# NickQrumpton/lattice-gaussian-mcmc

Hardware: AMD Instinct MI355X
Metric: Klein samples/sec at n=512 NTRU (IMHK proposals, d=1024) (higher is better)
Workload: dtype f64

## Files before the change

include/lgs.h:

```cpp
#ifndef LGS_H
#define LGS_H

#include <stdint.h>

#ifdef __cplusplus
extern "C" {
#endif

#define LGS_OK 0
#define LGS_ERR_INVALID (-1)
#define LGS_ERR_HIP (-2)
#define LGS_ERR_NOMEM (-3)
#define LGS_ERR_OVERFLOW (-4)
#define LGS_ERR_NONFINITE (-5)
#define LGS_ERR_STATE (-6)

#define LGS_BASIS_LINEAR_PROBS 0x1u

#define LGS_DEVICE_PTRS 0x1u
#define LGS_EXACT_ORDER 0x2u
#define LGS_WANG_LING 0x4u
#define LGS_Z64 0x8u
#define LGS_COORD_MAJOR 0x10u
#define LGS_SAMPLEZ_TABLE 0x20u
// ... 118 lines not shown
int lgs_timing_get(lgs_ctx *ctx, int kernel, double *ms_total, int64_t *launches);

#define LGS_COUNTER_RESOLVED 0
#define LGS_COUNTER_FALLBACK 1
#define LGS_COUNTER_ACCEPT_RESOLVED 2
#define LGS_COUNTER_WL_MISMATCH 3
#define LGS_COUNTER_QSKIP 4
#define LGS_COUNTER_KLEIN_CUS 5
#define LGS_COUNTER_DECODE_RESOLVED 6
#define LGS_COUNTER_LAUNCH_EXACT 7
#define LGS_COUNTER_LAUNCH_VALU 8
#define LGS_COUNTER_LAUNCH_MFMA_FP64 9
#define LGS_COUNTER_LAUNCH_MFMA_I8 10
int lgs_counter(lgs_ctx *ctx, int which, int reset, uint64_t *value);

int lgs_device_info(lgs_ctx *ctx, char *name, int name_len, int *n_cu, int64_t *hbm_bytes);

#ifdef __cplusplus
}
#endif
#endif
```

lattice-gaussian-mcmc_amd/csrc/lgs_capi.hip:

```cpp
#include <hip/hip_runtime.h>

#include <algorithm>
#include <cmath>
#include <cstdarg>
#include <cstdio>
#include <cstdlib>
#include <climits>
#include <cstring>
#include <string>
#include <vector>

#include "../../include/lgs.h"
#include "lgs_kernels.h"
#include "lgs_szc_host.h"

namespace {

thread_local std::string g_err;

int fail(int code, const char* fmt, ...) {
    char buf[512];
    va_list ap;
    va_start(ap, fmt);
    vsnprintf(buf, sizeof(buf), fmt, ap);
    va_end(ap);
    g_err = buf;
    return code;
}
// ... 14 lines not shown
static bool hook_is(const char* name, int v) {
    const char* e = hook(name);
    return e && atoi(e) == v;
}

#ifdef LGS_TEST_HOOKS
static size_t test_nomem_above() {
    const char* e = hook("LGS_TEST_NOMEM_ABOVE");
    return e ? (size_t)atoll(e) : 0;
}
#endif

struct DevBuf {
    void* p = nullptr;
    size_t bytes = 0;
    ~DevBuf() {
        if (p) (void)hipFree(p);
    }
    int reserve(size_t need) {
        if (need <= bytes) return LGS_OK;
        if (p) {
            (void)hipFree(p);
            p = nullptr;
            bytes = 0;
        }
        if (need == 0) return LGS_OK;
#ifdef LGS_TEST_HOOKS
        if (test_nomem_above() && need > test_nomem_above())
            return fail(LGS_ERR_NOMEM, "hipMalloc(%zu) refused (LGS_TEST_NOMEM_ABOVE)", need);
#endif
        hipError_t e = hipMalloc(&p, need);
        if (e != hipSuccess) {
            p = nullptr;
            return fail(LGS_ERR_NOMEM, "hipMalloc(%zu) failed: %s", need, hipGetErrorString(e));
        }
        bytes = need;
        return LGS_OK;
    }
    void release() {
        if (p) (void)hipFree(p);
        p = nullptr;
        bytes = 0;
    }
    template <typename T>
    T* as() const {
        return (T*)p;
    }
};

struct Timer {
    int kernel;
// ... 21 lines not shown
    int64_t d = 0;
    double sigma = 0;
    int precision = 10;
    uint32_t basis_flags = 0;
    int panel = 32;
    bool has_B = false;
    DevBuf R, RP, RC, BT, coord;
    DevBuf CREC, RX;
    DevBuf CERT;
    uint64_t n_resolved = 0;
    DevBuf RT, LWE, EMAX;
    DevBuf QZ2;
    bool has_qz2 = false;
    uint64_t n_accept_resolved = 0, n_wl_mismatch = 0;
    uint64_t n_qskip = 0;
    uint64_t n_decode_resolved = 0;
    uint64_t n_fallback = 0;
    uint64_t n_launch[4] = {};
    double z1cap = 0.0, z1seen = 0.0;
    unsigned int resolved_seen = 0;
    DevBuf RD, RDOFF;
    bool has_rd = false, oz_off = false;
    DevBuf H16, F0;
    DevBuf ZNZ;
    DevBuf CLIVE;
    DevBuf VNP;
    DevBuf LAGP;
    struct {
        const void* Z = nullptr;
        int64_t lanes = 0, cols = 0;
// ... 20 lines not shown
    int zint = 2;
    bool timing = false;
    double t_ms[9] = {0, 0, 0, 0, 0, 0, 0, 0, 0};
    int64_t t_n[9] = {0, 0, 0, 0, 0, 0, 0, 0, 0};
    DevBuf dg_x, dg_y, dg_out, dg_a, dg_b, dg_c, dg_t;
    DevBuf DQ, DBIT;
    DevBuf CPT;
    DevBuf DEC_D, DEC_E, DEC_WIN, DEC_BEST, DEC_D2, DEC_Z;
    bool has_q = false, has_binv = false;
    std::vector<Timer> pending;
    std::vector<hipEvent_t> pool;
    unsigned int* fw_host = nullptr;
    hipEvent_t fw_ev = nullptr;
    struct BlockSet {
        DevBuf Z, LW, H16, ZNZ, CLIVE, flags;
        hipEvent_t ev_free = nullptr;
        bool free_recorded = false;
    } bset[3];
    int bset_next = 0;
    int nsets = 2;
    bool kstream_sets_fixed = false;
    hipStream_t kstream = nullptr;
    hipStream_t kstream_full = nullptr, kstream_split = nullptr;
    int cu_split = 0;
    int kstream_cus = 0;
    int split_cus = 0;
    hipEvent_t kt0 = nullptr, kt1 = nullptr;
    bool kt_pending = false;
    double kt_bz_ms = 0.0;
    hipEvent_t ev_klein = nullptr;
// ... 5 lines not shown
        bool wl = false, exact = false, oz = false;
        decltype(hist) h;
        hipEvent_t ev = nullptr;
    } spec;
};

namespace {

int check_ctx(lgs_ctx* c, bool need_basis = true) {
    if (!c) return fail(LGS_ERR_INVALID, "null context");
    if (need_basis && c->d <= 0) return fail(LGS_ERR_STATE, "no basis loaded (lgs_set_basis)");
    HIP_TRY(hipSetDevice(c->device));
    return LGS_OK;
}

hipEvent_t get_event(lgs_ctx* c) {
    if (!c->pool.empty()) {
        hipEvent_t e = c->pool.back();
        c->pool.pop_back();
        return e;
    }
    hipEvent_t e = nullptr;
    (void)hipEventCreateWithFlags(&e, hipEventDisableSystemFence);
    return e;
}

struct Scope {
    lgs_ctx* c;
    int k;
    hipEvent_t a = nullptr;
// ... 5 lines not shown
    }
    ~Scope() {
        if (c->timing && a) {
            hipEvent_t b = get_event(c);
            (void)hipEventRecord(b, c->stream);
            c->pending.push_back({k, a, b});
        }
    }
};

int run_bz_fp64(lgs_ctx* c, const BzCall& b);

void swap_buf(DevBuf& a, DevBuf& b) {
    std::swap(a.p, b.p);
    std::swap(a.bytes, b.bytes);
}

struct SetSwap {
    lgs_ctx* c = nullptr;
    int j = -1;
    bool flags_in = false, store_in = false;
    void swap_flags() {
        swap_buf(c->flags, c->bset[j].flags);
        flags_in = !flags_in;
    }
    void swap_store() {
        auto& s = c->bset[j];
        swap_buf(c->Z, s.Z);
        swap_buf(c->LW, s.LW);
        swap_buf(c->H16, s.H16);
        swap_buf(c->ZNZ, s.ZNZ);
        swap_buf(c->CLIVE, s.CLIVE);
        store_in = !store_in;
    }
    void restore() {
        if (j < 0) return;
        if (store_in) swap_store();
        if (flags_in) swap_flags();
    }
    bool record = true;
    void release() {
        if (j < 0) return;
        restore();
        if (record) {
            (void)hipEventRecord(c->bset[j].ev_free, c->stream);
            c->bset[j].free_recorded = true;
        }
// ... 12 lines not shown
    const double cost = (double)ms * (double)(ncu - c->split_cus) / (double)c->split_cus;
    if (c->kt_bz_ms > cost) {
        HIP_TRY(hipStreamSynchronize(c->kstream_full));
        c->kstream = c->kstream_split;
        c->kstream_cus = c->split_cus;
        c->cu_split = 1;
    } else {
        c->cu_split = 2;
    }
    return LGS_OK;
}

int spec_discard(lgs_ctx* c) {
    if (!c->spec.valid) return LGS_OK;
    c->spec.valid = false;
    HIP_TRY(hipStreamSynchronize(c->kstream));
    HIP_TRY(hipMemset(c->bset[c->spec.j].flags.p, 0, 4 * lgs::kFlagWords));
    size_t keep = 0;
    for (auto& t : c->pending) {
        if (t.spec) {
            c->pool.push_back(t.a);
            c->pool.push_back(t.b);
        } else {
            c->pending[keep++] = t;
        }
    }
    c->pending.resize(keep);
    return LGS_OK;
}

// ... 51 lines not shown
    }
    c->pending.resize(keep);
}

int finish(lgs_ctx* c, const unsigned int* fw_known = nullptr, bool clear_all = false) {
    int rc0 = settle_bz(c, fw_known);
    if (rc0) return rc0;
    fold_timers(c);
    unsigned int fw[lgs::kFlagWords] = {};
    if (fw_known)
        memcpy(fw, fw_known, sizeof(fw));
    else
        HIP_TRY(hipMemcpy(fw, c->flags.p, sizeof(fw), hipMemcpyDeviceToHost));
    const unsigned int f = fw[0];
    c->resolved_seen = 0;
    if (fw[1] || fw[2] || fw[3])
        fold_counters(c, fw);
    c->n_accept_resolved += fw[lgs::kFlagWordAcceptResolved];
    c->n_wl_mismatch += fw[lgs::kFlagWordWLMismatch];
    c->n_qskip += fw[lgs::kFlagWordQSkip];
    c->n_decode_resolved += fw[lgs::kFlagWordDecodeResolved];
    bool any = false;
    for (int k = 1; k < lgs::kFlagWords; ++k) any |= fw[k] != 0;
    if (clear_all)
        HIP_TRY(hipMemsetAsync(c->flags.p, 0, lgs::kFlagWords * sizeof(unsigned int), c->stream));
    else if (any)
        HIP_TRY(hipMemsetAsync((unsigned int*)c->flags.p + 1, 0, (lgs::kFlagWords - 1) * sizeof(unsigned int),
                               c->stream));
    if (f & lgs::kFlagNonFinite)
        return fail(LGS_ERR_NONFINITE, "non-finite conditional mean (reference raises ValueError)");
    if (f & lgs::kFlagOverflow)
        return fail(LGS_ERR_OVERFLOW, "coefficient |z| >= 2^31: rerun with LGS_Z64");
    return LGS_OK;
}

int finish_or_redo(lgs_ctx* c, bool oz_used, int& zb, bool& redo, bool early = false) {
    redo = false;
    unsigned int fw[lgs::kFlagWords];
    if (early) {
        HIP_TRY(hipEventSynchronize(c->fw_ev));
        memcpy(fw, c->fw_host, sizeof(fw));
    } else {
        HIP_TRY(hipStreamSynchronize(c->stream));
        HIP_TRY(hipMemcpy(fw, c->flags.p, sizeof(fw), hipMemcpyDeviceToHost));
    }
    if (!(fw[0] & lgs::kAbortMask)) return finish(c, fw, early);
    c->pending_i8.clear();
    c->i8_dev_replay = false;
    for (auto& t : c->pending) {
        c->pool.push_back(t.a);
        c->pool.push_back(t.b);
    }
    c->pending.clear();
    c->n_fallback += 1;
    c->n_resolved += fw[kFlagWordCheckpoint];
    if (fw[0] & lgs::kFlagOverflow16) {
        if (zb == 2) c->zint = 4;
        if (oz_used) c->oz_off = true;
    }
    if (fw[0] & lgs::kFlagCarry16) c->zint = 4;
    if (zb == 2) zb = c->zint;
    HIP_TRY(hipMemsetAsync(c->flags.p, 0, 4 * lgs::kFlagWords, c->stream));
    redo = true;
    return LGS_OK;
}

int reset_flags(lgs_ctx* c) {
    int rc = c->flags.reserve(4 * lgs::kFlagWords);
    if (rc) return rc;
    c->resolved_seen = 0;
    HIP_TRY(hipMemsetAsync(c->flags.p, 0, 4 * lgs::kFlagWords, c->stream));
    return LGS_OK;
}

lgs::KleinArgs base_args(lgs_ctx* c, uint64_t seed) {
    lgs::KleinArgs a{};
    const double* co = c->coord.as<double>();
    const int64_t d = c->d;
    a.d = (int)d;
    a.precision = c->precision;
    a.linear_probs = (c->basis_flags & LGS_BASIS_LINEAR_PROBS) ? 1 : 0;
    a.cp = co;
    a.rii = co + d;
    a.sig = co + 2 * d;
// ... 53 lines not shown
        if ((rc = c->ZNZ.reserve((size_t)blocks * lanes))) return rc;
        a.znz = c->ZNZ.as<uint8_t>();
        if (c->d % 16 == 0) {
            const int64_t words = (c->d + 2047) / 2048 * (lanes / 64);
            if ((rc = c->CLIVE.reserve((size_t)words * 4))) return rc;
            HIP_TRY(hipMemsetAsync(c->CLIVE.p, 0, (size_t)words * 4, c->stream));
            a.clive = c->CLIVE.as<unsigned int>();
            a.clive_ld = lanes / 64;
        }
        a.rd = c->RD.as<int8_t>();
        a.rd_off = c->RDOFF.as<int64_t>();
        a.h16 = c->H16.as<int16_t>();
        a.h16_shift = shift;
        a.h16_lanes = lanes;
        used_oz = true;
    }
    const int launched = kernel == lgs::kKernelExact  ? LGS_COUNTER_LAUNCH_EXACT
                         : kernel == lgs::kKernelValu ? LGS_COUNTER_LAUNCH_VALU
                         : used_oz                    ? LGS_COUNTER_LAUNCH_MFMA_I8
                                                      : LGS_COUNTER_LAUNCH_MFMA_FP64;
    c->n_launch[launched - LGS_COUNTER_LAUNCH_EXACT] += 1;
    HIP_TRY(lgs::launch::klein(a, c->R.as<double>(), c->RP.as<double>(), c->RC.as<double>(),
                               c->panel, kernel, wl, zb, Z, c->stream));
    return LGS_OK;
}

int run_klein_store(lgs_ctx* c, lgs::KleinArgs& a, bool exact, bool wl, int& zb, void* Z, bool deferred,
                    bool* oz_out = nullptr) {
    bool oz = false;
    int rc = run_klein(c, a, exact, wl, zb, Z, oz);
// ... 285 lines not shown
    return LGS_OK;
}


int lgs_set_basis(lgs_ctx* c, int64_t d, const double* R, const double* cprime, const double* B,
                  double sigma, int32_t precision, uint32_t flags) {
    int rc = check_ctx(c, false);
    if (rc) return rc;
    if (d <= 0 || d > (1 << 20)) return fail(LGS_ERR_INVALID, "dimension %lld out of range", (long long)d);
    if (!R || !cprime) return fail(LGS_ERR_INVALID, "R and cprime are required");
    if (!(sigma > 0) || !std::isfinite(sigma))
        return fail(LGS_ERR_INVALID, "Standard deviation must be positive, got %g", sigma);
    if (precision <= 0) return fail(LGS_ERR_INVALID, "precision must be positive");
    HIP_TRY(hipStreamSynchronize(c->stream));
    if ((rc = spec_discard(c))) return rc;
    if (c->kstream_split && c->cu_split != 0 && !hook("LGS_PIPE_CU_RESERVE")) {
        HIP_TRY(hipStreamSynchronize(c->kstream));
        c->kstream = c->kstream_full;
        c->kstream_cus = 0;
        c->cu_split = 0;
    }
    c->kt_pending = false;
    const int PB = c->panel;
    const size_t dd = (size_t)d;
    std::vector<double> co(8 * dd);
    for (size_t i = 0; i < dd; ++i) {
        const double rii = R[i * dd + i];
        if (rii == 0.0 || !std::isfinite(rii))
            return fail(LGS_ERR_INVALID, "R[%zu,%zu] must be finite and non-zero", i, i);
        const double sref = sigma / std::fabs(rii);
// ... 366 lines not shown
    const int64_t d = c->d;
    const int zb = z64 ? 8 : 4;
    if ((rc = reset_flags(c))) return rc;
    const void* Zc = z;
    if (!dev || !cm) {
        if ((rc = c->Z.reserve((size_t)n * d * zb)) || (rc = c->stage_a.reserve((size_t)n * d * zb)))
            return rc;
        const void* src = z;
        if (!dev) {
            HIP_TRY(hipMemcpyAsync(c->stage_a.p, z, (size_t)n * d * zb, hipMemcpyHostToDevice, c->stream));
            src = c->stage_a.p;
        }
        if (cm) {
            Zc = src;
        } else {
            HIP_TRY(lgs::launch::to_coord_major(src, zb, n, (int)d, c->Z.p, zb, n, c->stream));
            Zc = c->Z.p;
        }
    }
    double* V = v_out;
    if (!dev) {
        if ((rc = c->V.reserve((size_t)n * d * 8))) return rc;
        V = c->V.as<double>();
    }
    if ((rc = run_bz(c, Zc, zb, n, n, V))) return rc;
    if ((rc = settle_bz(c))) return rc;
    if (!dev) HIP_TRY(hipMemcpyAsync(v_out, V, (size_t)n * d * 8, hipMemcpyDeviceToHost, c->stream));
    return finish(c);
}

// ... 6 lines not shown
    const int64_t d = c->d;
    const int zb = z64 ? 8 : 4;
    if ((rc = reset_flags(c))) return rc;
    const void* Zc = z;
    if (!dev || !cm) {
        if ((rc = c->Z.reserve((size_t)n * d * zb)) || (rc = c->stage_a.reserve((size_t)n * d * zb)))
            return rc;
        const void* src = z;
        if (!dev) {
            HIP_TRY(hipMemcpyAsync(c->stage_a.p, z, (size_t)n * d * zb, hipMemcpyHostToDevice, c->stream));
            src = c->stage_a.p;
        }
        if (cm) {
            Zc = src;
        } else {
            HIP_TRY(lgs::launch::to_coord_major(src, zb, n, (int)d, c->Z.p, zb, n, c->stream));
            Zc = c->Z.p;
        }
    }
    double* o = out;
    if (!dev) {
        if ((rc = c->LW.reserve((size_t)n * 8))) return rc;
        o = c->LW.as<double>();
    }
    lgs::KleinArgs a = base_args(c, 0);
    a.n = n;
    a.ldz = n;
    HIP_TRY(lgs::launch::log_density(a, c->R.as<double>(), Zc, zb, o, c->stream));
    if (!dev) HIP_TRY(hipMemcpyAsync(out, o, (size_t)n * 8, hipMemcpyDeviceToHost, c->stream));
    return finish(c);
// ... 545 lines not shown
        if (value) *value = (uint64_t)c->kstream_cus;
        return LGS_OK;
    }
    uint64_t& v = which >= LGS_COUNTER_LAUNCH_EXACT  ? c->n_launch[which - LGS_COUNTER_LAUNCH_EXACT]
                  : which == LGS_COUNTER_RESOLVED    ? c->n_resolved
                  : which == LGS_COUNTER_FALLBACK    ? c->n_fallback
                  : which == LGS_COUNTER_ACCEPT_RESOLVED ? c->n_accept_resolved
                  : which == LGS_COUNTER_WL_MISMATCH ? c->n_wl_mismatch
                  : which == LGS_COUNTER_DECODE_RESOLVED ? c->n_decode_resolved
                                                     : c->n_qskip;
    if (value) *value = v;
    if (reset) v = 0;
    return LGS_OK;
}

int lgs_device_info(lgs_ctx* c, char* name, int name_len, int* n_cu, int64_t* hbm) {
    int rc = check_ctx(c, false);
    if (rc) return rc;
    hipDeviceProp_t p;
    HIP_TRY(hipGetDeviceProperties(&p, c->device));
    if (name && name_len > 0) {
        snprintf(name, (size_t)name_len, "%s (%s)", p.name, p.gcnArchName);
    }
    if (n_cu) *n_cu = p.multiProcessorCount;
    if (hbm) *hbm = (int64_t)p.totalGlobalMem;
    return LGS_OK;
}

}

// ... 355 lines not shown
            for (int64_t i = 0; i < d; ++i)
                HIP_TRY(hipMemcpyAsync(X + (size_t)i * m, targets + (size_t)i * n + off, (size_t)m * 8,
                                       kind_of(true, dev), c->stream));
        } else {
            const double* src = targets + (size_t)off * d;
            if (!dev) {
                HIP_TRY(hipMemcpyAsync(c->stage_a.p, src, (size_t)m * d * 8, hipMemcpyHostToDevice, c->stream));
                src = c->stage_a.as<double>();
            }
            HIP_TRY(lgs::launch::to_coord_major(src, 8, m, (int)d, X, 8, m, c->stream));
        }
        HIP_TRY(lgs::launch::gemm_f64(X, m, plane ? c->DQ.as<double>() : c->DBIT.as<double>(), (int)d, m, Y,
                                      c->stream));
        HIP_TRY(lgs::launch::to_coord_major(Y, 8, m, (int)d, X, 8, m, c->stream));
        void* Zp = c->Z.p;
        if (plane) {
            const double* co = c->coord.as<double>();
            HIP_TRY(lgs::launch::nearest_plane((int)d, m, c->panel, c->RP.as<double>(), c->RC.as<double>(),
                                               co + d, X, m, ob, Zp, m, c->flags.as<unsigned int>(),
                                               c->stream));
        } else {
            HIP_TRY(lgs::launch::round_coeffs(X, m, (int)d, m, ob, Zp, m, c->flags.as<unsigned int>(),
                                              c->stream));
        }
        if (z_out) {
            if (cm) {
                for (int64_t i = 0; i < d; ++i)
                    HIP_TRY(hipMemcpyAsync((char*)z_out + ((size_t)i * n + off) * ob, (char*)Zp + (size_t)i * m * ob,
                                           (size_t)m * ob, kind_of(dev, true), c->stream));
            } else {
// ... 112 lines not shown
                }
                if (!qframe) {
                    HIP_TRY(lgs::launch::gemm_f64(c->dg_x.as<double>(), m, c->DQ.as<double>(), (int)d, m,
                                                  c->dg_y.as<double>(), c->stream));
                    src = c->dg_y.as<double>();
                }
                HIP_TRY(lgs::launch::to_coord_major(src, 8, m, (int)d, X, 8, mp, c->stream));
            }
        }
        lgs::KleinArgs a = base_args(c, seed);
        a.counter_mode = 0;
        a.base = first + (uint64_t)off;
        a.n = mp;
        a.ldz = mp;
        void* Zp = c->Z.p;
        {
            Scope s(c, 0);
            c->hist.Z = nullptr;
            HIP_TRY(lgs::launch::klein_targets(a, c->R.as<double>(), c->RP.as<double>(), c->RC.as<double>(), c->panel,
                                               exact, X, mp, dmu_scale, ob, Zp, c->stream));
        }
        if (z_out) {
            if (cm) {
                HIP_TRY(hipMemcpy2DAsync((char*)z_out + (size_t)off * ob, (size_t)n * ob, Zp, (size_t)mp * ob,
                                         (size_t)m * ob, (size_t)d, kind_of(dev, true), c->stream));
            } else {
                void* dst = dev ? (char*)z_out + (size_t)off * d * ob : c->stage_a.p;
                HIP_TRY(lgs::launch::transpose_out(Zp, ob, mp, m, (int)d, dst, ob, c->stream));
                if (!dev)
                    HIP_TRY(hipMemcpyAsync((char*)z_out + (size_t)off * d * ob, dst, (size_t)m * d * ob,
// ... 90 lines not shown
                }
                if (!qframe) {
                    HIP_TRY(lgs::launch::gemm_f64(c->dg_x.as<double>(), m, c->DQ.as<double>(), (int)d, m,
                                                  c->dg_y.as<double>(), c->stream));
                    src = c->dg_y.as<double>();
                }
                HIP_TRY(lgs::launch::to_coord_major(src, 8, m, (int)d, X, 8, ldc, c->stream));
            }
        }
        lgs::KleinArgs a = base_args(c, seed);
        a.counter_mode = 0;
        a.base = first + (uint64_t)off * (uint64_t)K;
        a.n = mp;
        a.ldz = mp;
        void* Zp = c->Z.p;
        const lgs::DecodeLanes dl{K, c->DEC_D.as<double>(), c->DEC_E.as<double>()};
        {
            Scope s(c, 0);
            c->hist.Z = nullptr;
            HIP_TRY(lgs::launch::klein_decode(a, c->R.as<double>(), c->RP.as<double>(), c->RC.as<double>(), c->panel,
                                              exact, X, ldc, dmu_scale, ob, Zp, dl, c->stream));
        }
        int64_t* best = dev && o.best_draw ? o.best_draw + off : c->DEC_BEST.as<int64_t>();
        double* dist2 = dev && o.dist2 ? o.dist2 + off : c->DEC_D2.as<double>();
        void* Wp = c->DEC_Z.p;
        {
            Scope s(c, 8);
            HIP_TRY(lgs::launch::decode_select((int)d, m, K, dl.D, dl.E, c->RT.as<double>(), X, ldc, Zp, ob, mp,
                                               c->DEC_WIN.as<int64_t>(), best, dist2, c->flags.as<unsigned int>(),
                                               c->stream, stage_ok));
// ... 44 lines not shown
```

lattice-gaussian-mcmc_amd/csrc/lgs_kernels.h:

```cpp
#pragma once
#include <hip/hip_runtime.h>
#include <stdint.h>


namespace lgs {

constexpr unsigned int kFlagNonFinite = 1u;
constexpr unsigned int kFlagOverflow = 2u;
constexpr unsigned int kFlagI8Range = 4u;
constexpr unsigned int kFlagOverflow16 = 8u;
constexpr unsigned int kFlagCarry16 = 16u;
constexpr unsigned int kAbortMask = kFlagOverflow16 | kFlagCarry16;
constexpr int kFlagWordResolved = 1;
constexpr int kFlagWordUninit = 4;
constexpr int kFlagWordCheckpoint = 5;

constexpr int kErfTabLast = 512;
constexpr int kCoefStride = 18;

constexpr int kSzDeg = 5;
constexpr int kSzS = 9;
constexpr int kSzB = kSzS + kSzDeg + 1;
constexpr int kSzCa = kSzB + kSzDeg + 1;
constexpr int kSzCb = kSzCa + 1;
// ... 54 lines not shown
    const double* cert;
    const double* crec;
    const int8_t* rd;
    const int64_t* rd_off;
    int16_t* h16;
    int h16_shift;
    int64_t h16_lanes;
    uint8_t* znz;
    const double* rx;
    const unsigned int* gate;
    double* LWE;
    unsigned long long* emax;
    const double* qz2;
    unsigned int* clive;
    int64_t clive_ld;
};

constexpr int kFlagWordAcceptResolved = 6;
constexpr int kFlagWordWLMismatch = 7;
constexpr int kFlagWordQSkip = 8;
constexpr int kFlagWordDecodeResolved = 9;
constexpr int kFlagWords = 16;

struct DecodeLanes {
    int64_t K;
    double* D;
    double* E;
};

struct AcceptArgs {
    int64_t nc;
    int64_t T;
    int64_t thin;
    int64_t n_keep;
    uint64_t seed;
    uint32_t chain0;
// ... 150 lines not shown
```

lattice-gaussian-mcmc_amd/csrc/lgs_kernels.hip:

```cpp
#include <hip/hip_runtime.h>

#include <type_traits>
#include <stdint.h>

#include "lgs_device.h"
#include "lgs_kernels.h"

namespace lgs {

typedef unsigned int v4u_t __attribute__((ext_vector_type(4)));

__device__ __forceinline__ void lane_counter(const KleinArgs& a, int64_t p, uint32_t& chain,
                                             uint32_t& step) {
    if (a.counter_mode == 0) {
        const uint64_t s = a.base + (uint64_t)p;
        chain = (uint32_t)s;
        step = (uint32_t)(s >> 32);
    } else {
        chain = a.chain0 + (uint32_t)(p / a.nt);
        step = a.step0 + (uint32_t)(p % a.nt);
    }
}

__device__ __forceinline__ double ref_weight(double zi, double mu, double ros, double isr, double lterm) {
// ... 803 lines not shown
#pragma unroll
    for (int g = 0; g < 4; ++g)
#pragma unroll
        for (int reg = 0; reg < 4; ++reg) F[(4 * h + reg) * LDF + 16 * g + n] = t0v[g][reg];
#ifdef LGS_DIAG_FAR
    {
        LGS_DF_T(tf_end);
        df[7] += 1;
        df[5] += (tf_end - tf_begin) - df[0] - df[1] - df[2] - df[3] - df[4];
        if ((threadIdx.x & 63) == 0)
            for (int k = 0; k < 8; ++k) atomicAdd(&lgs_diag_far[k], (unsigned long long)df[k]);
    }
#endif
}

#ifdef LGS_DIAG_CYCLES
__device__ unsigned long long lgs_diag_cycles[16];
#define LGS_DC_T(v) const uint64_t v = __builtin_amdgcn_s_memtime()
#define LGS_DC_ADD(k, x) dc[k] += (x)
#else
#define LGS_DC_T(v)
#define LGS_DC_ADD(k, x)
#endif
constexpr int kOzLB = 2, kMfmaLB32 = 3;
template <typename ZT, int PB, bool WL, bool OZ = false, bool LIBM = false>
__global__ __launch_bounds__(256, PB == 32 ? (OZ ? kOzLB : kMfmaLB32) : 3) void klein_mfma_kernel(const KleinArgs a,
                                                            const double* __restrict__ RP,
                                                            const double* __restrict__ RC,
                                                            ZT* __restrict__ Z) {
    if (a.gate && *a.gate == 0u) return;
    constexpr int NT = PB / 16, LDF = 65;
    __shared__ double Fl[4][16 * LDF];
    __shared__ double tab_lds[OZ ? 2 : 2 * (kErfTabLast + 1)];
    __shared__ __attribute__((aligned(16))) int8_t ash[OZ ? 2 * 2 * kOzDigits * 1024 : 16];
    using ETP = std::conditional_t<OZ, gdptr, lds_cdptr>;
    ETP etab_s;
    if constexpr (OZ)
        etab_s = (gdptr)a.etab;
    else
        etab_s = stage_etab(tab_lds, a.etab);
    __shared__ __attribute__((aligned(16))) double rec_lds[PB == 32 ? 32 * kRecStride : 2];
    __shared__ uint32_t nzm[OZ ? kOzMaxD / 32 / 32 : 1];
    if constexpr (OZ)
        for (int e = threadIdx.x; e < kOzMaxD / 32 / 32; e += 256) nzm[e] = 0u;
    const int lane = threadIdx.x & 63, wave = threadIdx.x >> 6;
#ifdef LGS_DIAG_CYCLES
    uint64_t dc[16] = {};
#endif
    LGS_DC_T(t_kernel0);
    const int64_t p0 = ((int64_t)blockIdx.x * 4 + wave) * 64;
    const bool active = p0 < a.n;
    if (!active && PB != 32) return;
    const int64_t p = p0 + lane;
    uint32_t chain, step;
    lane_counter(a, p, chain, step);
    CoordStream rs;
    rs.init(a.seed, step, chain);
// ... 32 lines not shown
            __syncthreads();
            const bool skip = qtry && __builtin_amdgcn_readfirstlane(qvote[pk & 1][0] & qvote[pk & 1][1] &
                                                                     qvote[pk & 1][2] & qvote[pk & 1][3]) != 0;
            if (!skip) {
                const double2* __restrict__ src = (const double2*)a.crec;
                double2* dst = (double2*)rec_lds;
                for (int e = threadIdx.x; e < 32 * kRecStride / 2; e += 256)
                    if (r0 * (kRecStride / 2) + e >= 0) dst[e] = src[(int64_t)r0 * (kRecStride / 2) + e];
                __syncthreads();
            }
            if (!active) continue;
            if (skip) {
                if (lane == 0) atomicAdd(a.flags + kFlagWordQSkip, 1u);
                const cdptr lt = uniformize(cst(a.lterm) + r0);
                double ltv[32];
#pragma unroll
                for (int s = 0; s < 32; ++s) ltv[s] = lt[31 - s];
#pragma unroll
                for (int s = 0; s < 32; ++s) {
                    Z[(size_t)(p_hi - 1 - s) * ldz + p] = (ZT)0;
                    lw += ltv[s];
                }
                v4u_t* hp4 = (v4u_t*)(a.h16 + ((size_t)((p_hi - 32 + a.h16_shift) >> 4) * a.h16_lanes + p) * 16);
                const v4u_t h128 = (v4u_t){0x00800080u, 0x00800080u, 0x00800080u, 0x00800080u};
                hp4[0] = h128;
                hp4[1] = h128;
                hp4[(size_t)a.h16_lanes * 2] = h128;
                hp4[(size_t)a.h16_lanes * 2 + 1] = h128;
                if (a.znz) {
                    a.znz[(size_t)((p_hi - 32 + a.h16_shift) >> 4) * a.h16_lanes + p] = 0;
                    a.znz[(size_t)((p_hi - 16 + a.h16_shift) >> 4) * a.h16_lanes + p] = 0;
                }
                continue;
            }
        }
        bool coarse = false;
        if constexpr (OZ && PB == 32 && !WL)
            coarse = p_hi >= 32 &&
                     __builtin_amdgcn_readfirstlane((int)((lds_cdptr)rec_lds)[31 * kRecStride + kRecSpec]) == 1 &&
                     __builtin_amdgcn_readfirstlane((int)((lds_cdptr)rec_lds)[15 * kRecStride + kRecSpec]) == 1;
        LGS_DC_T(t_far0);
        LGS_DC_ADD(0, t_far0 - t_panel0);
        if (pk > 0) {
            __builtin_amdgcn_fence(__ATOMIC_RELEASE, "wavefront");
            __builtin_amdgcn_wave_barrier();
          if constexpr (OZ && PB == 32) {
            oz_far_field(a, pk, p_hi, p0, lane, (lds_cdptr)rec_lds, F, LDF, acc, ash, nzm, coarse);
            (void)NT;
// ... 322 lines not shown
    }
    if constexpr (PB == 32) {
        double m = active ? cert_lds[0][threadIdx.x] : 0.0;
#pragma unroll
        for (int o = 32; o >= 1; o >>= 1) m = fmax(m, __shfl_xor(m, o));
        if (lane == 0 && a.z1max) atomicMax(a.z1max, (unsigned long long)__double_as_longlong(m));
    }
    const double ewl = WL ? wl_bound_sum(eb, tb, d) : 0.0;
    if (WL && PB == 32 && a.emax) {
        double m = active ? ewl : 0.0;
#pragma unroll
        for (int o = 32; o >= 1; o >>= 1) m = fmax(m, __shfl_xor(m, o));
        if (lane == 0) atomicMax(a.emax, (unsigned long long)__double_as_longlong(m));
    }
    if (!active) return;
    if (a.LW) a.LW[p] = lw;
    if (WL && PB == 32 && a.LWE) a.LWE[p] = ewl;
    if (WL && PB != 32) wl_bound_store(a, p, ewl);
    if (flags) atomicOr(a.flags, flags);
#ifdef LGS_DIAG_CYCLES
    LGS_DC_T(t_kernel1);
    dc[13] = t_kernel1 - t_kernel0;
    if (lane == 0)
        for (int k = 0; k < 16; ++k) atomicAdd(&lgs_diag_cycles[k], (unsigned long long)dc[k]);
#endif
}


template <typename ZT>
__device__ __forceinline__ double resolve_coord(const KleinArgs& a, int i, double cpl, const ZT* Zp, size_t ldz,
// ... 1493 lines not shown
            __VA_ARGS__;                   \
        } else {                           \
            using T = int64_t;             \
            __VA_ARGS__;                   \
        }                                  \
    } while (0)

template <typename ZT, int PB>
static void klein_pb(const KleinArgs& a, const double* RP, const double* RC, int kernel, bool wl,
                     ZT* z, dim3 grid, hipStream_t st) {
    if (kernel == kKernelMfma) {
        const bool libm = a.szc == nullptr;
        if (PB == 32 && a.rd) {
            if (libm && wl)
                hipLaunchKernelGGL((klein_mfma_kernel<ZT, PB, true, true, true>), grid, dim3(256), 0, st, a, RP, RC, z);
            else if (libm)
                hipLaunchKernelGGL((klein_mfma_kernel<ZT, PB, false, true, true>), grid, dim3(256), 0, st, a, RP, RC, z);
            else if (wl)
                hipLaunchKernelGGL((klein_mfma_kernel<ZT, PB, true, true>), grid, dim3(256), 0, st, a, RP, RC, z);
            else
                hipLaunchKernelGGL((klein_mfma_kernel<ZT, PB, false, true>), grid, dim3(256), 0, st, a, RP, RC, z);
        } else if (libm && wl)
            hipLaunchKernelGGL((klein_mfma_kernel<ZT, PB, true, false, true>), grid, dim3(256), 0, st, a, RP, RC, z);
        else if (libm)
            hipLaunchKernelGGL((klein_mfma_kernel<ZT, PB, false, false, true>), grid, dim3(256), 0, st, a, RP, RC, z);
        else if (wl)
            hipLaunchKernelGGL((klein_mfma_kernel<ZT, PB, true>), grid, dim3(256), 0, st, a, RP, RC, z);
        else
            hipLaunchKernelGGL((klein_mfma_kernel<ZT, PB, false>), grid, dim3(256), 0, st, a, RP, RC, z);
    } else {
        if (wl)
// ... 394 lines not shown
```

lattice-gaussian-mcmc_amd/lgs_amd/_capi.py:

```python
from __future__ import annotations

import ctypes
import os

import numpy as np

_HERE = os.path.dirname(os.path.abspath(__file__))
LIB_PATH = os.environ.get("LGS_LIB") or os.path.join(_HERE, "_lib", "liblgs_hip.so")
HOOKS_LIB_PATH = os.path.join(_HERE, "_lib", "liblgs_hip_hooks.so")

LGS_OK = 0
LGS_ERR_INVALID = -1
LGS_ERR_HIP = -2
LGS_ERR_NOMEM = -3
LGS_ERR_OVERFLOW = -4
LGS_ERR_NONFINITE = -5
LGS_ERR_STATE = -6

LGS_BASIS_LINEAR_PROBS = 0x1
LGS_DEVICE_PTRS = 0x1
LGS_EXACT_ORDER = 0x2
LGS_WANG_LING = 0x4
LGS_Z64 = 0x8
LGS_COORD_MAJOR = 0x10
# ... 23 lines not shown
LGS_COUNTER_FALLBACK = 1
LGS_COUNTER_ACCEPT_RESOLVED = 2
LGS_COUNTER_WL_MISMATCH = 3
LGS_COUNTER_QSKIP = 4
LGS_COUNTER_KLEIN_CUS = 5
LGS_COUNTER_DECODE_RESOLVED = 6
LGS_COUNTER_LAUNCH_EXACT = 7
LGS_COUNTER_LAUNCH_VALU = 8
LGS_COUNTER_LAUNCH_MFMA_FP64 = 9
LGS_COUNTER_LAUNCH_MFMA_I8 = 10

EXPORTS = ("lgs_version", "lgs_last_error", "lgs_create", "lgs_create_ex", "lgs_destroy", "lgs_set_stream",
           "lgs_set_basis", "lgs_klein", "lgs_imhk", "lgs_imhk_trace", "lgs_imhk_ex", "lgs_lattice_points", "lgs_log_density", "lgs_sample_z", "lgs_timing_enable",
           "lgs_timing_get", "lgs_device_info", "lgs_series_stats", "lgs_gram",
           "lgs_jump_distance", "lgs_marginal_tvd", "lgs_column_range", "lgs_histogram", "lgs_set_decoder", "lgs_nearest_plane",
           "lgs_round_decode", "lgs_counter", "lgs_klein_targets", "lgs_klein_decode")


class ImhkOutputs(ctypes.Structure):
    _fields_ = [("logw_samples", ctypes.c_void_p), ("accepted", ctypes.c_void_p),
                ("vnorm2_samples", ctypes.c_void_p), ("zk_samples", ctypes.c_void_p),
                ("zk_index", ctypes.c_int64), ("fn_chains", ctypes.c_int64),
                ("lag_L", ctypes.c_int64), ("lag_z_ring", ctypes.c_void_p), ("lag_z_sums", ctypes.c_void_p),
                ("lag_v_ring", ctypes.c_void_p), ("lag_v_sums", ctypes.c_void_p), ("lag_v_scale", ctypes.c_double)]


class DecodeOutputs(ctypes.Structure):
    _fields_ = [("best_draw", ctypes.c_void_p), ("dist2", ctypes.c_void_p),
                ("dist2_draws", ctypes.c_void_p), ("bound_draws", ctypes.c_void_p)]


# ... 39 lines not shown
                           ctypes.c_uint32]
    L.lgs_imhk_trace.argtypes = [_vp, ctypes.c_uint64, ctypes.c_uint64, ctypes.c_int64, ctypes.c_uint64,
                                 ctypes.c_int64, ctypes.c_int32, _vp, _vp, _vp, _vp, _vp, _vp, _vp,
                                 _vp, _vp, ctypes.c_uint32]
    if hasattr(L, "lgs_imhk_ex"):
        L.lgs_imhk_ex.argtypes = [_vp, ctypes.c_uint64, ctypes.c_uint64, ctypes.c_int64, ctypes.c_uint64,
                                  ctypes.c_int64, ctypes.c_int32, _vp, _vp, _vp, _vp, _vp, _vp, _vp,
                                  ctypes.POINTER(ImhkOutputs), ctypes.c_uint32]
    L.lgs_lattice_points.argtypes = [_vp, ctypes.c_int64, _vp, _vp, ctypes.c_uint32]
    L.lgs_log_density.argtypes = [_vp, ctypes.c_int64, _vp, _vp, ctypes.c_uint32]
    L.lgs_sample_z.argtypes = [_vp, ctypes.c_int64, _vp, _vp, _vp, ctypes.c_int32, _vp, _vp,
                               ctypes.c_uint32]
    L.lgs_timing_enable.argtypes = [_vp, ctypes.c_int]
    L.lgs_timing_get.argtypes = [_vp, ctypes.c_int, _dp, _i64p]
    L.lgs_counter.argtypes = [_vp, ctypes.c_int, ctypes.c_int, ctypes.POINTER(ctypes.c_uint64)]
    L.lgs_device_info.argtypes = [_vp, ctypes.c_char_p, ctypes.c_int, ctypes.POINTER(ctypes.c_int),
                                  _i64p]
    _i64 = ctypes.c_int64
    L.lgs_series_stats.argtypes = [_vp, _vp, _i64, _i64, _i64, _i64, _i64, _i64, _i64,
                                   ctypes.c_double, _i64, _vp, _vp, _vp, _vp, _vp, ctypes.c_uint32]
    L.lgs_gram.argtypes = [_vp, _i64, _i64, _vp, _i64, _vp, _vp, _vp, ctypes.c_uint32]
    L.lgs_jump_distance.argtypes = [_vp, _i64, _i64, _vp, _i64, _vp, ctypes.c_uint32]
    L.lgs_marginal_tvd.argtypes = [_vp, _i64, _vp, _i64, _vp, _i64, _vp, ctypes.c_uint32]
    L.lgs_column_range.argtypes = [_vp, _i64, _vp, _i64, _vp, _vp, ctypes.c_uint32]
    L.lgs_histogram.argtypes = [_vp, _i64, _vp, _i64, _i64, _vp, _vp, _vp, ctypes.c_uint32]
    L.lgs_set_decoder.argtypes = [_vp, _vp, _vp]
    L.lgs_nearest_plane.argtypes = [_vp, _i64, _vp, _vp, _vp, ctypes.c_uint32]
    L.lgs_round_decode.argtypes = [_vp, _i64, _vp, _vp, _vp, ctypes.c_uint32]
    if hasattr(L, "lgs_klein_targets"):
        L.lgs_klein_targets.argtypes = [_vp, ctypes.c_uint64, ctypes.c_uint64, _i64, _vp, _vp, _vp, _vp,
# ... 378 lines not shown
    def resolved(self, reset=False):
        v = ctypes.c_uint64(0)
        self._ck(self._L.lgs_counter(self._h, LGS_COUNTER_RESOLVED, 1 if reset else 0, ctypes.byref(v)))
        return v.value

    def fallbacks(self, reset=False):
        v = ctypes.c_uint64(0)
        self._ck(self._L.lgs_counter(self._h, LGS_COUNTER_FALLBACK, 1 if reset else 0, ctypes.byref(v)))
        return v.value

    def counter(self, which, reset=False):
        v = ctypes.c_uint64(0)
        self._ck(self._L.lgs_counter(self._h, int(which), 1 if reset else 0, ctypes.byref(v)))
        return v.value

    def device_info(self):
        buf = ctypes.create_string_buffer(256)
        ncu = ctypes.c_int(0)
        mem = ctypes.c_int64(0)
        self._ck(self._L.lgs_device_info(self._h, buf, 256, ctypes.byref(ncu), ctypes.byref(mem)))
        return {"name": buf.value.decode(), "n_cu": ncu.value, "hbm_bytes": mem.value}


def version() -> int:
    return load_library().lgs_version()
```

Baseline: 124.3 million.

## Track per-panel clean state to skip redundant zero stores on quick-skip panels

Adds a per-(chain block, panel) byte map recording that the Z, H16 and ZNZ regions for a quick-skipped panel were already zeroed by a previous launch. On later launches with the same buffers, basis and layout (validated by a host-side key with buffer ids and a gate flag), the kernel skips rewriting those zeros. It still accumulates the log-weight terms. This targets global store traffic in the far-field skip path. In exchange it adds host-side invalidation bookkeeping across many entry points and an extra kernel template variant, and it relies on every buffer mutation being tracked correctly.

```diff
diff --git a/include/lgs.h b/include/lgs.h
--- a/include/lgs.h
+++ b/include/lgs.h
@@ -156,6 +156,8 @@
 #define LGS_COUNTER_LAUNCH_MFMA_I8 10
 int lgs_counter(lgs_ctx *ctx, int which, int reset, uint64_t *value);
 
+int lgs_qskip_elided(lgs_ctx *ctx, int reset, uint64_t *value);
+
 int lgs_device_info(lgs_ctx *ctx, char *name, int name_len, int *n_cu, int64_t *hbm_bytes);
 
 #ifdef __cplusplus
diff --git a/lattice-gaussian-mcmc_amd/csrc/lgs_capi.hip b/lattice-gaussian-mcmc_amd/csrc/lgs_capi.hip
--- a/lattice-gaussian-mcmc_amd/csrc/lgs_capi.hip
+++ b/lattice-gaussian-mcmc_amd/csrc/lgs_capi.hip
@@ -1,6 +1,7 @@
 #include <hip/hip_runtime.h>
 
 #include <algorithm>
+#include <atomic>
 #include <cmath>
 #include <cstdarg>
 #include <cstdio>
@@ -12,6 +13,7 @@
 
 #include "../../include/lgs.h"
 #include "lgs_kernels.h"
+#include "lgs_qclean_host.h"
 #include "lgs_szc_host.h"
 
 namespace {
@@ -56,6 +58,7 @@
 struct DevBuf {
     void* p = nullptr;
     size_t bytes = 0;
+    uint64_t id = 0;
     ~DevBuf() {
         if (p) (void)hipFree(p);
     }
@@ -77,6 +80,8 @@
             return fail(LGS_ERR_NOMEM, "hipMalloc(%zu) failed: %s", need, hipGetErrorString(e));
         }
         bytes = need;
+        static std::atomic<uint64_t> serial{0};
+        id = ++serial;
         return LGS_OK;
     }
     void release() {
@@ -128,6 +133,10 @@
     bool has_qz2 = false;
     uint64_t n_accept_resolved = 0, n_wl_mismatch = 0;
     uint64_t n_qskip = 0;
+    uint64_t n_qskip_elided = 0;
+    DevBuf QCL;
+    lgs::QKey qkey;
+    uint64_t basis_gen = 0;
     uint64_t n_decode_resolved = 0;
     uint64_t n_fallback = 0;
     uint64_t n_launch[4] = {};
@@ -178,6 +187,8 @@
     hipEvent_t fw_ev = nullptr;
     struct BlockSet {
         DevBuf Z, LW, H16, ZNZ, CLIVE, flags;
+        DevBuf QCL;
+        lgs::QKey qkey;
         hipEvent_t ev_free = nullptr;
         bool free_recorded = false;
     } bset[3];
@@ -213,6 +224,11 @@
     return LGS_OK;
 }
 
+void qclean_flags_cleared(lgs_ctx* c) {
+    lgs::qkey_flags_cleared(c->qkey);
+    for (auto& s : c->bset) lgs::qkey_flags_cleared(s.qkey);
+}
+
 hipEvent_t get_event(lgs_ctx* c) {
     if (!c->pool.empty()) {
         hipEvent_t e = c->pool.back();
@@ -248,6 +264,7 @@
 void swap_buf(DevBuf& a, DevBuf& b) {
     std::swap(a.p, b.p);
     std::swap(a.bytes, b.bytes);
+    std::swap(a.id, b.id);
 }
 
 struct SetSwap {
@@ -265,6 +282,8 @@
         swap_buf(c->H16, s.H16);
         swap_buf(c->ZNZ, s.ZNZ);
         swap_buf(c->CLIVE, s.CLIVE);
+        swap_buf(c->QCL, s.QCL);
+        std::swap(c->qkey, s.qkey);
         store_in = !store_in;
     }
     void restore() {
@@ -307,6 +326,8 @@
 int spec_discard(lgs_ctx* c) {
     if (!c->spec.valid) return LGS_OK;
     c->spec.valid = false;
+    lgs::qkey_drop(c->bset[c->spec.j].qkey);
+    qclean_flags_cleared(c);
     HIP_TRY(hipStreamSynchronize(c->kstream));
     HIP_TRY(hipMemset(c->bset[c->spec.j].flags.p, 0, 4 * lgs::kFlagWords));
     size_t keep = 0;
@@ -388,11 +409,13 @@
         HIP_TRY(hipMemcpy(fw, c->flags.p, sizeof(fw), hipMemcpyDeviceToHost));
     const unsigned int f = fw[0];
     c->resolved_seen = 0;
+    qclean_flags_cleared(c);
     if (fw[1] || fw[2] || fw[3])
         fold_counters(c, fw);
     c->n_accept_resolved += fw[lgs::kFlagWordAcceptResolved];
     c->n_wl_mismatch += fw[lgs::kFlagWordWLMismatch];
     c->n_qskip += fw[lgs::kFlagWordQSkip];
+    c->n_qskip_elided += fw[lgs::kFlagWordQSkipElided];
     c->n_decode_resolved += fw[lgs::kFlagWordDecodeResolved];
     bool any = false;
     for (int k = 1; k < lgs::kFlagWords; ++k) any |= fw[k] != 0;
@@ -419,6 +442,7 @@
         HIP_TRY(hipMemcpy(fw, c->flags.p, sizeof(fw), hipMemcpyDeviceToHost));
     }
     if (!(fw[0] & lgs::kAbortMask)) return finish(c, fw, early);
+    qclean_flags_cleared(c);
     c->pending_i8.clear();
     c->i8_dev_replay = false;
     for (auto& t : c->pending) {
@@ -442,6 +466,7 @@
 int reset_flags(lgs_ctx* c) {
     int rc = c->flags.reserve(4 * lgs::kFlagWords);
     if (rc) return rc;
+    qclean_flags_cleared(c);
     c->resolved_seen = 0;
     HIP_TRY(hipMemsetAsync(c->flags.p, 0, 4 * lgs::kFlagWords, c->stream));
     return LGS_OK;
@@ -525,6 +550,37 @@
         a.h16_shift = shift;
         a.h16_lanes = lanes;
         used_oz = true;
+    }
+    a.qclean = nullptr;
+    a.qclean_reset = 0;
+    a.qclean_gate = nullptr;
+    const int64_t npan = (c->d + 31) / 32;
+    if (used_oz && !wl && a.qz2 && !a.gate && Z == c->Z.p && npan <= lgs::kQCleanPanels) {
+        const int rc = c->QCL.reserve(((size_t)(a.h16_lanes / 64) * npan + 3) / 4 * 4);
+        if (rc) return rc;
+        lgs::QKey k;
+        k.z_id = c->Z.id;
+        k.h16_id = c->H16.id;
+        k.znz_id = c->ZNZ.id;
+        k.state_id = c->QCL.id;
+        k.Z = Z;
+        k.H16 = a.h16;
+        k.ZNZ = a.znz;
+        k.ldz = a.ldz;
+        k.h16_lanes = a.h16_lanes;
+        k.n = a.n;
+        k.h16_shift = a.h16_shift;
+        k.d = a.d;
+        k.zb = zb;
+        k.counter_mode = a.counter_mode;
+        k.chain0 = a.chain0;
+        k.basis_gen = c->basis_gen;
+        a.qclean = c->QCL.as<uint8_t>();
+        a.qclean_reset = lgs::qkey_claim(c->qkey, k, &a.qclean_gate) ? 0 : 1;
+    } else if (a.gate && Z == c->Z.p) {
+        lgs::qkey_gated_write(c->qkey, a.gate);
+    } else {
+        lgs::qkey_drop(c->qkey);
     }
     const int launched = kernel == lgs::kKernelExact  ? LGS_COUNTER_LAUNCH_EXACT
                          : kernel == lgs::kKernelValu ? LGS_COUNTER_LAUNCH_VALU
@@ -840,6 +896,9 @@
     if (precision <= 0) return fail(LGS_ERR_INVALID, "precision must be positive");
     HIP_TRY(hipStreamSynchronize(c->stream));
     if ((rc = spec_discard(c))) return rc;
+    c->basis_gen += 1;
+    lgs::qkey_drop(c->qkey);
+    for (auto& s : c->bset) lgs::qkey_drop(s.qkey);
     if (c->kstream_split && c->cu_split != 0 && !hook("LGS_PIPE_CU_RESERVE")) {
         HIP_TRY(hipStreamSynchronize(c->kstream));
         c->kstream = c->kstream_full;
@@ -1236,6 +1295,7 @@
         if (cm) {
             Zc = src;
         } else {
+            lgs::qkey_drop(c->qkey);
             HIP_TRY(lgs::launch::to_coord_major(src, zb, n, (int)d, c->Z.p, zb, n, c->stream));
             Zc = c->Z.p;
         }
@@ -1272,6 +1332,7 @@
         if (cm) {
             Zc = src;
         } else {
+            lgs::qkey_drop(c->qkey);
             HIP_TRY(lgs::launch::to_coord_major(src, zb, n, (int)d, c->Z.p, zb, n, c->stream));
             Zc = c->Z.p;
         }
@@ -1847,6 +1908,13 @@
     return LGS_OK;
 }
 
+int lgs_qskip_elided(lgs_ctx* c, int reset, uint64_t* value) {
+    if (!c) return fail(LGS_ERR_INVALID, "null context");
+    if (value) *value = c->n_qskip_elided;
+    if (reset) c->n_qskip_elided = 0;
+    return LGS_OK;
+}
+
 int lgs_device_info(lgs_ctx* c, char* name, int name_len, int* n_cu, int64_t* hbm) {
     int rc = check_ctx(c, false);
     if (rc) return rc;
@@ -2232,6 +2300,7 @@
                                       c->stream));
         HIP_TRY(lgs::launch::to_coord_major(Y, 8, m, (int)d, X, 8, m, c->stream));
         void* Zp = c->Z.p;
+        lgs::qkey_drop(c->qkey);
         if (plane) {
             const double* co = c->coord.as<double>();
             HIP_TRY(lgs::launch::nearest_plane((int)d, m, c->panel, c->RP.as<double>(), c->RC.as<double>(),
@@ -2374,6 +2443,7 @@
         a.n = mp;
         a.ldz = mp;
         void* Zp = c->Z.p;
+        lgs::qkey_drop(c->qkey);
         {
             Scope s(c, 0);
             c->hist.Z = nullptr;
@@ -2494,6 +2564,7 @@
         a.n = mp;
         a.ldz = mp;
         void* Zp = c->Z.p;
+        lgs::qkey_drop(c->qkey);
         const lgs::DecodeLanes dl{K, c->DEC_D.as<double>(), c->DEC_E.as<double>()};
         {
             Scope s(c, 0);
diff --git a/lattice-gaussian-mcmc_amd/csrc/lgs_kernels.h b/lattice-gaussian-mcmc_amd/csrc/lgs_kernels.h
--- a/lattice-gaussian-mcmc_amd/csrc/lgs_kernels.h
+++ b/lattice-gaussian-mcmc_amd/csrc/lgs_kernels.h
@@ -92,12 +92,17 @@
     const double* qz2;
     unsigned int* clive;
     int64_t clive_ld;
-};
+    uint8_t* qclean;
+    int qclean_reset;
+    const unsigned int* qclean_gate;
+};
+constexpr int kQCleanPanels = 128;
 
 constexpr int kFlagWordAcceptResolved = 6;
 constexpr int kFlagWordWLMismatch = 7;
 constexpr int kFlagWordQSkip = 8;
 constexpr int kFlagWordDecodeResolved = 9;
+constexpr int kFlagWordQSkipElided = 10;
 constexpr int kFlagWords = 16;
 
 struct DecodeLanes {
diff --git a/lattice-gaussian-mcmc_amd/csrc/lgs_kernels.hip b/lattice-gaussian-mcmc_amd/csrc/lgs_kernels.hip
--- a/lattice-gaussian-mcmc_amd/csrc/lgs_kernels.hip
+++ b/lattice-gaussian-mcmc_amd/csrc/lgs_kernels.hip
@@ -841,6 +841,11 @@
 #endif
 }
 
+__device__ __forceinline__ bool qclean_reset(const KleinArgs& a) {
+    return a.qclean_reset != 0 ||
+           (a.qclean_gate != nullptr && *(const __attribute__((address_space(4))) unsigned int*)a.qclean_gate != 0u);
+}
+
 #ifdef LGS_DIAG_CYCLES
 __device__ unsigned long long lgs_diag_cycles[16];
 #define LGS_DC_T(v) const uint64_t v = __builtin_amdgcn_s_memtime()
@@ -850,7 +855,7 @@
 #define LGS_DC_ADD(k, x)
 #endif
 constexpr int kOzLB = 2, kMfmaLB32 = 3;
-template <typename ZT, int PB, bool WL, bool OZ = false, bool LIBM = false>
+template <typename ZT, int PB, bool WL, bool OZ = false, bool LIBM = false, bool QC = false>
 __global__ __launch_bounds__(256, PB == 32 ? (OZ ? kOzLB : kMfmaLB32) : 3) void klein_mfma_kernel(const KleinArgs a,
                                                             const double* __restrict__ RP,
                                                             const double* __restrict__ RC,
@@ -868,6 +873,10 @@
         etab_s = stage_etab(tab_lds, a.etab);
     __shared__ __attribute__((aligned(16))) double rec_lds[PB == 32 ? 32 * kRecStride : 2];
     __shared__ uint32_t nzm[OZ ? kOzMaxD / 32 / 32 : 1];
+    static_assert(!QC || (OZ && !WL && PB == 32), "clean state: int8-digit far field, reference mode");
+    __shared__ uint32_t qcnt[QC ? 4 : 1];
+    if constexpr (QC)
+        if (threadIdx.x < 4) qcnt[threadIdx.x] = 0u;
     if constexpr (OZ)
         for (int e = threadIdx.x; e < kOzMaxD / 32 / 32; e += 256) nzm[e] = 0u;
     const int lane = threadIdx.x & 63, wave = threadIdx.x >> 6;
@@ -930,12 +939,29 @@
                 if (lane == 0) atomicAdd(a.flags + kFlagWordQSkip, 1u);
                 const cdptr lt = uniformize(cst(a.lterm) + r0);
                 double ltv[32];
-#pragma unroll
-                for (int s = 0; s < 32; ++s) ltv[s] = lt[31 - s];
-#pragma unroll
-                for (int s = 0; s < 32; ++s) {
-                    Z[(size_t)(p_hi - 1 - s) * ldz + p] = (ZT)0;
-                    lw += ltv[s];
+                if constexpr (QC) {
+                    uint32_t qcw = 0u;
+                    const uint32_t qi = (uint32_t)__builtin_amdgcn_readfirstlane((int)(p0 >> 6)) * (uint32_t)npan + pk;
+                    if (!qclean_reset(a)) qcw = ((const __attribute__((address_space(4))) uint32_t*)a.qclean)[qi >> 2];
+#pragma unroll
+                    for (int s = 0; s < 32; ++s) ltv[s] = lt[31 - s];
+#pragma unroll
+                    for (int s = 0; s < 32; ++s) lw += ltv[s];
+                    if (((qcw >> (8 * (qi & 3))) & 0xffu) != 0u) {
+                        if (lane == 0) qcnt[wave] += 1u;
+                        continue;
+                    }
+                    if (lane == 0) a.qclean[qi] = 1;
+#pragma unroll
+                    for (int s = 0; s < 32; ++s) Z[(size_t)(p_hi - 1 - s) * ldz + p] = (ZT)0;
+                } else {
+#pragma unroll
+                    for (int s = 0; s < 32; ++s) ltv[s] = lt[31 - s];
+#pragma unroll
+                    for (int s = 0; s < 32; ++s) {
+                        Z[(size_t)(p_hi - 1 - s) * ldz + p] = (ZT)0;
+                        lw += ltv[s];
+                    }
                 }
                 v4u_t* hp4 = (v4u_t*)(a.h16 + ((size_t)((p_hi - 32 + a.h16_shift) >> 4) * a.h16_lanes + p) * 16);
                 const v4u_t h128 = (v4u_t){0x00800080u, 0x00800080u, 0x00800080u, 0x00800080u};
@@ -948,6 +974,9 @@
                     a.znz[(size_t)((p_hi - 16 + a.h16_shift) >> 4) * a.h16_lanes + p] = 0;
                 }
                 continue;
+            }
+            if constexpr (QC) {
+                if ((qtry || qclean_reset(a)) && lane == 0) a.qclean[(uint32_t)(p0 >> 6) * (uint32_t)npan + pk] = 0;
             }
         }
         bool coarse = false;
@@ -1300,6 +1329,9 @@
         if (lane == 0) atomicMax(a.emax, (unsigned long long)__double_as_longlong(m));
     }
     if (!active) return;
+    if constexpr (QC) {
+        if (lane == 0 && qcnt[wave] != 0u) atomicAdd(a.flags + kFlagWordQSkipElided, qcnt[wave]);
+    }
     if (a.LW) a.LW[p] = lw;
     if (WL && PB == 32 && a.LWE) a.LWE[p] = ewl;
     if (WL && PB != 32) wl_bound_store(a, p, ewl);
@@ -2823,7 +2855,13 @@
         if (PB == 32 && a.rd) {
             if (libm && wl)
                 hipLaunchKernelGGL((klein_mfma_kernel<ZT, PB, true, true, true>), grid, dim3(256), 0, st, a, RP, RC, z);
-            else if (libm)
+            else if (PB == 32 && a.qclean && !wl) {
+                constexpr bool QC = PB == 32;
+                if (libm)
+                    hipLaunchKernelGGL((klein_mfma_kernel<ZT, PB, false, true, true, QC>), grid, dim3(256), 0, st, a, RP, RC, z);
+                else
+                    hipLaunchKernelGGL((klein_mfma_kernel<ZT, PB, false, true, false, QC>), grid, dim3(256), 0, st, a, RP, RC, z);
+            } else if (libm)
                 hipLaunchKernelGGL((klein_mfma_kernel<ZT, PB, false, true, true>), grid, dim3(256), 0, st, a, RP, RC, z);
             else if (wl)
                 hipLaunchKernelGGL((klein_mfma_kernel<ZT, PB, true, true>), grid, dim3(256), 0, st, a, RP, RC, z);
diff --git a/lattice-gaussian-mcmc_amd/csrc/lgs_qclean_host.h b/lattice-gaussian-mcmc_amd/csrc/lgs_qclean_host.h
--- /dev/null
+++ b/lattice-gaussian-mcmc_amd/csrc/lgs_qclean_host.h
@@ -0,0 +1,48 @@
+#pragma once
+#include <cstdint>
+
+namespace lgs {
+
+struct QKey {
+    bool valid = false;
+    uint64_t z_id = 0, h16_id = 0, znz_id = 0, state_id = 0;
+    const void* Z = nullptr;
+    const void* H16 = nullptr;
+    const void* ZNZ = nullptr;
+    int64_t ldz = 0, h16_lanes = 0, n = 0;
+    int h16_shift = 0, d = 0, zb = 0;
+    int counter_mode = 0;
+    uint32_t chain0 = 0;
+    uint64_t basis_gen = 0;
+    const unsigned int* dirty_if = nullptr;
+
+    bool same(const QKey& o) const {
+        return z_id == o.z_id && h16_id == o.h16_id && znz_id == o.znz_id && state_id == o.state_id && Z == o.Z &&
+               H16 == o.H16 && ZNZ == o.ZNZ && ldz == o.ldz && h16_lanes == o.h16_lanes && n == o.n &&
+               h16_shift == o.h16_shift && d == o.d && zb == o.zb && counter_mode == o.counter_mode &&
+               chain0 == o.chain0 && basis_gen == o.basis_gen;
+    }
+};
+
+inline bool qkey_claim(QKey& cur, const QKey& launch, const unsigned int** gate) {
+    const bool trusted = cur.valid && cur.same(launch);
+    *gate = trusted ? cur.dirty_if : nullptr;
+    cur = launch;
+    cur.valid = true;
+    cur.dirty_if = nullptr;
+    return trusted;
+}
+
+inline void qkey_gated_write(QKey& cur, const unsigned int* gate) {
+    if (cur.dirty_if != nullptr && cur.dirty_if != gate) cur.valid = false;
+    cur.dirty_if = gate;
+}
+
+inline void qkey_flags_cleared(QKey& cur) {
+    if (cur.dirty_if != nullptr) cur.valid = false;
+    cur.dirty_if = nullptr;
+}
+
+inline void qkey_drop(QKey& cur) { cur.valid = false; }
+
+}
diff --git a/lattice-gaussian-mcmc_amd/lgs_amd/_capi.py b/lattice-gaussian-mcmc_amd/lgs_amd/_capi.py
--- a/lattice-gaussian-mcmc_amd/lgs_amd/_capi.py
+++ b/lattice-gaussian-mcmc_amd/lgs_amd/_capi.py
@@ -61,7 +61,7 @@
            "lgs_set_basis", "lgs_klein", "lgs_imhk", "lgs_imhk_trace", "lgs_imhk_ex", "lgs_lattice_points", "lgs_log_density", "lgs_sample_z", "lgs_timing_enable",
            "lgs_timing_get", "lgs_device_info", "lgs_series_stats", "lgs_gram",
            "lgs_jump_distance", "lgs_marginal_tvd", "lgs_column_range", "lgs_histogram", "lgs_set_decoder", "lgs_nearest_plane",
-           "lgs_round_decode", "lgs_counter", "lgs_klein_targets", "lgs_klein_decode")
+           "lgs_round_decode", "lgs_counter", "lgs_qskip_elided", "lgs_klein_targets", "lgs_klein_decode")
 
 
 class ImhkOutputs(ctypes.Structure):
@@ -131,6 +131,7 @@
     L.lgs_timing_enable.argtypes = [_vp, ctypes.c_int]
     L.lgs_timing_get.argtypes = [_vp, ctypes.c_int, _dp, _i64p]
     L.lgs_counter.argtypes = [_vp, ctypes.c_int, ctypes.c_int, ctypes.POINTER(ctypes.c_uint64)]
+    L.lgs_qskip_elided.argtypes = [_vp, ctypes.c_int, ctypes.POINTER(ctypes.c_uint64)]
     L.lgs_device_info.argtypes = [_vp, ctypes.c_char_p, ctypes.c_int, ctypes.POINTER(ctypes.c_int),
                                   _i64p]
     _i64 = ctypes.c_int64
@@ -539,6 +540,11 @@
         self._ck(self._L.lgs_counter(self._h, int(which), 1 if reset else 0, ctypes.byref(v)))
         return v.value
 
+    def qskip_elided(self, reset=False):
+        v = ctypes.c_uint64(0)
+        self._ck(self._L.lgs_qskip_elided(self._h, 1 if reset else 0, ctypes.byref(v)))
+        return v.value
+
     def device_info(self):
         buf = ctypes.create_string_buffer(256)
         ncu = ctypes.c_int(0)
```

Result: faster. 127.6 million, median of 6 (+2.7%).
